# josiahbjorgaard/mca-paper

Measured on AMD Instinct MI355X. Metric: training samples/sec (fwd+bwd+opt), CMU 4-modality MCA, higher is better.
Workload: dtype bf16; 1 GPU; synthetic CMU 4-modality (MCA fcl), N=2538 D=512 L=5 H=8 F=88, lengths=full, p_drop=0.0; per_gpu_batch=32, global_batch=32, parallelism=dp1, inputs=device-resident, same batch every step, finite_checks=on (device flag, polled), attention_operands=bf16, attention_backward=bf16 one-pass, launch=hipGraph replay (one launch per step), collectives=none

## Files before the change

include/mca_hip.h:

```cpp
#ifndef MCA_HIP_H
#define MCA_HIP_H
#include <stdint.h>

#ifdef __cplusplus
extern "C" {
#endif

typedef void* mca_stream_t;

#define MCA_OK 0
#define MCA_E_BADARG (-1)
#define MCA_E_ALIGN (-2)
#define MCA_E_UNSUPPORTED (-3)
#define MCA_E_LAUNCH (-4)

const char* mca_version(void);

int mca_gemm_nt(const uint16_t* A, int64_t lda, const uint16_t* B, int64_t ldb,
                void* C, int64_t ldc, int out_bf16,
                const float* bias, const float* residual, int64_t ldres, int64_t res_period,
                int64_t M, int64_t N, int64_t K, mca_stream_t stream);

int mca_gemm_nt_cb(const uint16_t* A, int64_t lda, const uint16_t* B, int64_t ldb, uint16_t* C, int64_t cbs,
                   int64_t M, int64_t N, int64_t K, mca_stream_t stream);
// ... 5 lines not shown
int mca_gemm_nt_geglu_bwd(const uint16_t* A, int64_t lda, const uint16_t* B, int64_t ldb, const uint16_t* h,
                          uint16_t* dh, int64_t ldh, int64_t ip, int64_t M, int64_t K, mca_stream_t stream);

int mca_gemm_nt_geglu_fwd(const uint16_t* A, int64_t lda, const uint16_t* W1, int64_t ldb, uint16_t* h, int64_t ldh,
                          uint16_t* g, int64_t ldg, int64_t ip, int64_t M, int64_t K, mca_stream_t stream);

int mca_gemm_nt_geglu_fwd_saved(const uint16_t* A, int64_t lda, const uint16_t* W1, int64_t ldb, uint16_t* s, int64_t lds,
                                uint16_t* g, int64_t ldg, int64_t ip, int64_t M, int64_t K, mca_stream_t stream);
int mca_gemm_nt_geglu_bwd_saved(const uint16_t* A, int64_t lda, const uint16_t* B, int64_t ldb, const uint16_t* s,
                                uint16_t* dh, int64_t ldh, int64_t ip, int64_t M, int64_t K, mca_stream_t stream);

int mca_gemm_nt_res_lnbwd(const uint16_t* A, int64_t lda, const uint16_t* B, int64_t ldb, const float* residual, int64_t ldres,
                          const float* x, int64_t ldx, const float* mean, const float* rstd, const float* gamma,
                          float* dx, int64_t lddx, uint16_t* dx_bf16, int64_t ld_bf16, float* dgamma,
                          int64_t M, int64_t N, int64_t K, mca_stream_t stream);

int mca_gemm_tn_acc(const uint16_t* A, int64_t lda, const uint16_t* B, int64_t ldb,
                    float* C, int64_t ldc, int64_t R, int64_t N, int64_t K, mca_stream_t stream);

#define MCA_TN_MAX_GROUP 8
typedef struct mca_tn_desc {
  const uint16_t* A; int64_t lda;
  const uint16_t* B; int64_t ldb;
  float* C; int64_t ldc;
  int64_t N, K;
} mca_tn_desc;
int mca_gemm_tn_acc_group(const mca_tn_desc* d, int n, int64_t R, mca_stream_t stream);

int mca_layernorm_fwd(const float* x, int64_t ldx, const float* gamma, const float* beta,
                      const uint8_t* rowmask, const float* add, int64_t period,
// ... 310 lines not shown
```

mca-paper_amd/csrc/gemm.hip:

```cpp
#include "common.h"
#include "gemm_plan.h"
#include "gemm_tile.h"
#include "ln_rows.h"

static int num_cus() {
  static int n = 0;
  if (!n) {
    int dev = 0;
    if (hipGetDevice(&dev) != hipSuccess || hipDeviceGetAttribute(&n, hipDeviceAttributeMultiprocessorCount, dev) != hipSuccess || n <= 0) n = 256;
  }
  return n;
}

#define PS_PANELS 4
__device__ __forceinline__ void ps_tile_decode(int tile, int tiles_m, int tiles_n, int flat, int& tm, int& tn) {
  if (flat == 1) { tm = tile / tiles_n; tn = tile % tiles_n; return; }
  const int P = flat > 1 ? flat : PS_PANELS;
  const int per_group = P * tiles_n;
  const int g = tile / per_group;
  const int gh = (g + 1) * P <= tiles_m ? P : tiles_m - g * P;
  const int rem = tile - g * per_group;
  tn = rem / gh; tm = g * P + rem % gh;
}

// ... 846 lines not shown
          st4b(dx_bf16 + r1 * ld_bf16 + c, o);
        }
      }
    }
  }
  __syncthreads();
#pragma unroll
  for (int i = 0; i < 2; i++) *reinterpret_cast<float4*>(cs + wave * ROWS_N + (lane + 64 * i) * 4) = dg[i];
  __syncthreads();
  float t = cs[tid];
#pragma unroll
  for (int w = 1; w < 8; w++) t += cs[w * ROWS_N + tid];
  if (t != 0.f) atomicAdd(dgamma + tid, t);
}


template <bool DET>
__global__ __launch_bounds__(256) void gemm_tn_kernel(const u16* __restrict__ A, int64_t lda,
                                                       const u16* __restrict__ B, int64_t ldb, float* __restrict__ C,
                                                       int64_t ldc, int R, int N, int K, int tiles_k, int rows_per_split, int dbg) {
  __shared__ __attribute__((aligned(16))) u16 lds[2 * 2 * BR * 128];
  u16* As = lds;
  u16* Bs = lds + 2 * BR * 128;
  const int tn = blockIdx.x / tiles_k, tk = blockIdx.x % tiles_k;
  const int n0 = tn * 128, k0 = tk * 128;
  const int r_begin = blockIdx.y * rows_per_split;
  int r_end = r_begin + rows_per_split; if (r_end > R) r_end = R;
  if (r_begin >= r_end) return;
  const int tid = threadIdx.x, lane = tid & 63, wave = tid >> 6;
  const int wn = wave >> 1, wk = wave & 1;
// ... 401 lines not shown
}

extern "C" int mca_gemm_nt_lnres(const uint16_t* A, int64_t lda, const uint16_t* B, int64_t ldb, float* C, int64_t ldc,
                                 const float* x, int64_t ldx, const float* mean, const float* rstd, const float* gamma,
                                 int64_t M, int64_t N, int64_t K, mca_stream_t stream) {
  if (!A || !B || !C || !x || !mean || !rstd || !gamma || M <= 0 || N <= 0 || K <= 0) return MCA_E_BADARG;
  if (K % 64 || lda % 8 || ldb % 8 || ldc % 4 || ldx % 4 || (uintptr_t)A % 16 || (uintptr_t)B % 16 || (uintptr_t)C % 16 ||
      (uintptr_t)x % 16 || (uintptr_t)gamma % 16)
    return MCA_E_ALIGN;
  if (lda < K || ldb < K || ldc < N || ldx < N) return MCA_E_BADARG;
  if (!mca_nt_lnres_supported(M, N, K)) return MCA_E_UNSUPPORTED;
  const gemm_operands o = {A, lda, B, ldb, C, ldc, nullptr, x, ldx, 0, mean, rstd, gamma, (int)M, (int)K, nullptr};
  return launch(mca_plan_gemm_nt_lnres(M, N), o, stream);
}

extern "C" int mca_gemm_nt_res_lnbwd(const uint16_t* A, int64_t lda, const uint16_t* B, int64_t ldb, const float* residual, int64_t ldres,
                                     const float* x, int64_t ldx, const float* mean, const float* rstd, const float* gamma,
                                     float* dx, int64_t lddx, uint16_t* dx_bf16, int64_t ld_bf16, float* dgamma,
                                     int64_t M, int64_t N, int64_t K, mca_stream_t stream) {
  if (!A || !B || !x || !mean || !rstd || !gamma || !dx || !dx_bf16 || !dgamma || M <= 0 || N <= 0 || K <= 0) return MCA_E_BADARG;
  const int refusal = mca_nt_rows_refusal(M, N, K);
  if (refusal) return refusal;
  if (lda % 8 || ldb % 8 || ldx % 4 || lddx % 4 || ld_bf16 % 8 || (residual && ldres % 4) || (uintptr_t)A % 16 || (uintptr_t)B % 16 ||
      (uintptr_t)x % 16 || (uintptr_t)gamma % 16 || (uintptr_t)dx % 16 || (uintptr_t)dx_bf16 % 16 || (uintptr_t)residual % 16)
    return MCA_E_ALIGN;
  if (lda < K || ldb < K || ldx < N || lddx < N || ld_bf16 < N || (residual && ldres < N)) return MCA_E_BADARG;
  const mca_gemm_plan p = mca_plan_gemm_nt_res_lnbwd(M);
  return launch_kernel<gemm_nt_rows_kernel>(p, stream, A, lda, B, ldb, residual, ldres, x, ldx, mean, rstd, gamma, dx, lddx, dx_bf16, ld_bf16,
                                               dgamma, (int)M, (int)K, p.nwg);
}

static int geglu_bwd_entry(bool saved, const uint16_t* A, int64_t lda, const uint16_t* B, int64_t ldb, const uint16_t* h,
                           uint16_t* dh, int64_t ldh, int64_t ip, int64_t M, int64_t K, mca_stream_t stream) {
  if (!A || !B || !h || !dh || M <= 0 || ip <= 0 || K <= 0) return MCA_E_BADARG;
  if (K % 64 || lda % 8 || ldb % 8 || ldh % 8 || ip % 8 || (uintptr_t)A % 16 || (uintptr_t)B % 16 || (uintptr_t)h % 16 || (uintptr_t)dh % 16)
    return MCA_E_ALIGN;
  if (lda < K || ldb < K || ldh < 2 * ip) return MCA_E_BADARG;
  if (M > (1LL << 30)) return MCA_E_UNSUPPORTED;
  const gemm_operands o = {A, lda, B, ldb, dh, ldh, nullptr, reinterpret_cast<const float*>(h), ldh, 0, nullptr, nullptr, nullptr, (int)M, (int)K, nullptr};
  return launch(saved ? mca_plan_gemm_nt_geglu_bwd_saved(M, ip, K, mca_knobs, num_cus()) : mca_plan_gemm_nt_geglu_bwd(M, ip, K, mca_knobs, num_cus()),
                o, stream);
}
extern "C" int mca_gemm_nt_geglu_bwd(const uint16_t* A, int64_t lda, const uint16_t* B, int64_t ldb, const uint16_t* h,
                                     uint16_t* dh, int64_t ldh, int64_t ip, int64_t M, int64_t K, mca_stream_t stream) {
// ... 160 lines not shown
  if (!pr || !out) return MCA_E_BADARG;
  if (cus <= 0) cus = num_cus();
  switch (entry) {
    case 0: *out = mca_plan_gemm_nt(*pr, mca_knobs, cus); return MCA_OK;
    case 1:
      if (!mca_nt_lnres_supported(pr->M, pr->N, pr->K)) return MCA_E_UNSUPPORTED;
      *out = mca_plan_gemm_nt_lnres(pr->M, pr->N); return MCA_OK;
    case 2: *out = mca_plan_gemm_nt_geglu_fwd(pr->M, pr->N, pr->K, mca_knobs, cus); return MCA_OK;
    case 3: *out = mca_plan_gemm_nt_geglu_bwd(pr->M, pr->N, pr->K, mca_knobs, cus); return MCA_OK;
    case 4: *out = mca_plan_gemm_nt_geglu_fwd_saved(pr->M, pr->N, pr->K, mca_knobs, cus); return MCA_OK;
    case 5: *out = mca_plan_gemm_nt_geglu_bwd_saved(pr->M, pr->N, pr->K, mca_knobs, cus); return MCA_OK;
    case 6:
      if (pr->M <= 0 || pr->N <= 0 || pr->K <= 0) return MCA_E_BADARG;
      if (mca_nt_rows_refusal(pr->M, pr->N, pr->K)) return mca_nt_rows_refusal(pr->M, pr->N, pr->K);
      *out = mca_plan_gemm_nt_res_lnbwd(pr->M); return MCA_OK;
  }
  return MCA_E_BADARG;
}
extern "C" int mca_dbg_plan_gemm_nt_cb(int64_t M, int64_t N, int64_t K, uint64_t C, int64_t cbs, int cus, mca_gemm_plan* out) {
  if (!out || M <= 0 || N <= 0 || K <= 0) return MCA_E_BADARG;
  if (cus <= 0) cus = num_cus();
  return mca_plan_gemm_nt_cb(M, N, K, C, cbs, mca_knobs, cus, out) ? MCA_OK : MCA_E_UNSUPPORTED;
}
extern "C" const char* mca_dbg_gemm_kernel_name(int kernel) { return mca_gemm_kernel_name(kernel); }
extern "C" int mca_dbg_plan_gemm_tn(int64_t R, int64_t N, int64_t K, mca_gemm_plan* out) {
  if (!out || R <= 0 || N <= 0 || K <= 0) return MCA_E_BADARG;
  *out = mca_plan_gemm_tn(R, N, K, mca_knobs);
  return MCA_OK;
}
extern "C" int mca_dbg_plan_gemm_tn_group(const int64_t* N, const int64_t* K, int n, int64_t R, int cus, mca_tn_group_plan* out) {
// ... 22 lines not shown
```

mca-paper_amd/csrc/gemm_plan.h:

```cpp
#pragma once
#include <stdint.h>

#define BM 128
#define BN 128
#define BM2 256
#define BR 64
#define BR2 32
#define P2_STAGE (512 * 32)
#define TN2_STAGE (BR2 * 512)
#define TN2_NSTAGE 5
#define NT256_LDS_BYTES (3 * (BM2 + BN) * 64 * 2)
#define NT256LN_LDS_BYTES (NT256_LDS_BYTES + 2048)
#define NTPS_LDS_BYTES (3 * (BM2 + BN) * 64 * 2 + 16384)
#define P2_LDS_BYTES (5 * P2_STAGE * 2)
#define TN256_LDS_BYTES (3 * BR * (256 + 128) * 2)
#define TN2_LDS_BYTES (TN2_NSTAGE * TN2_STAGE * 2)

enum mca_gemm_kernel {
  MCA_GK_NONE = 0,
  MCA_GK_NT_GLDS = 1,
  MCA_GK_NT_GLDS_GEGLU_BWD = 7,
  MCA_GK_NT_256 = 8,
  MCA_GK_NT_256_PF = 14,
  MCA_GK_NT_256_LNRES = 15,
// ... 3 lines not shown
  MCA_GK_NT_PERSIST_GEGLU_FWD = 24,
  MCA_GK_NT_PERSIST256 = 25,
  MCA_GK_NT_PERSIST256_GEGLU_FWD = 26,
  MCA_GK_TN = 27,
  MCA_GK_TN_256 = 28,
  MCA_GK_TN_256X256 = 29,
  MCA_GK_TN_256X256_GROUP = 30,
  MCA_GK_COUNT = 31,
  MCA_GK_SAVED = 64,
  MCA_GK_NT_GLDS_GEGLU_BWD_SAVED = MCA_GK_SAVED + MCA_GK_NT_GLDS_GEGLU_BWD,
  MCA_GK_NT_256_GEGLU_BWD_SAVED = MCA_GK_SAVED + MCA_GK_NT_256_GEGLU_BWD,
  MCA_GK_NT_PERSIST_GEGLU_BWD_SAVED = MCA_GK_SAVED + MCA_GK_NT_PERSIST_GEGLU_BWD,
  MCA_GK_NT_PERSIST_GEGLU_FWD_SAVED = MCA_GK_SAVED + MCA_GK_NT_PERSIST_GEGLU_FWD,
  MCA_GK_NT_PERSIST256_GEGLU_FWD_SAVED = MCA_GK_SAVED + MCA_GK_NT_PERSIST256_GEGLU_FWD,
  MCA_GK_NT_ROWS_LNBWD = 128,
  MCA_GK_NT_PERSIST256_CB = 256
};

static inline const char* mca_gemm_kernel_name(int k) {
  static const char* const names[MCA_GK_COUNT] = {
      "none",
      "gemm_nt_glds_kernel<false,0,64,0>", "gemm_nt_glds_kernel<false,1,64,0>", "gemm_nt_glds_kernel<false,2,64,0>",
      "gemm_nt_glds_kernel<true,0,64,0>", "gemm_nt_glds_kernel<true,1,64,0>", "gemm_nt_glds_kernel<true,2,64,0>",
      "gemm_nt_glds_kernel<true,0,64,1>",
      "gemm_nt_256_kernel<false,0,0,0>", "gemm_nt_256_kernel<false,1,0,0>", "gemm_nt_256_kernel<false,2,0,0>",
      "gemm_nt_256_kernel<true,0,0,0>", "gemm_nt_256_kernel<true,1,0,0>", "gemm_nt_256_kernel<true,2,0,0>",
      "gemm_nt_256_kernel<false,1,1,0>", "gemm_nt_256_kernel<false,1,1,2>", "gemm_nt_256_kernel<true,0,0,1>",
      "gemm_nt_persist_kernel<0,false>", "gemm_nt_persist_kernel<0,true>", "gemm_nt_persist_kernel<1,false>",
      "gemm_nt_persist_kernel<1,true>", "gemm_nt_persist_kernel<2,false>", "gemm_nt_persist_kernel<2,true>",
      "gemm_nt_persist_kernel<3,false>", "gemm_nt_persist_kernel<4,false>",
      "gemm_nt_persist256_kernel<false>", "gemm_nt_persist256_kernel<true>",
      "gemm_tn_kernel", "gemm_tn_256_kernel", "gemm_tn_256x256_kernel", "gemm_tn_256x256_group_kernel"};
  switch (k) {
    case MCA_GK_NT_GLDS_GEGLU_BWD_SAVED: return "gemm_nt_glds_kernel<true,0,64,3>";
    case MCA_GK_NT_256_GEGLU_BWD_SAVED: return "gemm_nt_256_kernel<true,0,0,3>";
    case MCA_GK_NT_PERSIST_GEGLU_BWD_SAVED: return "gemm_nt_persist_kernel<5,false>";
    case MCA_GK_NT_PERSIST_GEGLU_FWD_SAVED: return "gemm_nt_persist_kernel<6,false>";
    case MCA_GK_NT_PERSIST256_GEGLU_FWD_SAVED: return "gemm_nt_persist256_kernel<true,true>";
    case MCA_GK_NT_ROWS_LNBWD: return "gemm_nt_rows_kernel";
    case MCA_GK_NT_PERSIST256_CB: return "gemm_nt_persist256_kernel<false,false,true>";
  }
  return k >= 0 && k < MCA_GK_COUNT ? names[k] : "?";
}

struct mca_gemm_plan {
  int kernel;
  int grid_x, grid_y, block, lds_bytes;
  int n;
  int tiles_n, nwg;
  int tiles_k, rows_per_split;
  int dbg;
};

#define MCA_NT_BIG_M 2048
// ... 124 lines not shown
#define ROWS_CS_LD (ROWS_N + 4)
#define ROWS_LDS_BYTES (ROWS_NSTAGE * ROWS_STAGE * 2)
#define MCA_NT_ROWS_MIN_K (ROWS_NSTAGE * ROWS_BK)

static inline int mca_nt_rows_refusal(int64_t M, int64_t N, int64_t K) {
  if (N != ROWS_N || M > (1LL << 30)) return -3;
  if (K % ROWS_BK) return -2;
  if (K < MCA_NT_ROWS_MIN_K) return -3;
  return 0;
}
static inline mca_gemm_plan mca_plan_gemm_nt_res_lnbwd(int64_t M) {
  mca_gemm_plan pl = {};
  pl.kernel = MCA_GK_NT_ROWS_LNBWD;
  pl.n = ROWS_N; pl.tiles_n = 1; pl.nwg = (int)((M + ROWS_BM - 1) / ROWS_BM);
  pl.grid_x = pl.nwg; pl.grid_y = 1; pl.block = 512; pl.lds_bytes = ROWS_LDS_BYTES;
  return pl;
}

#define MCA_TN_BIG_N 512
#define MCA_TN_BIG_R 4096
#define MCA_TN_HUGE_MIN_K 512
#define MCA_TN_HUGE_MIN_TILES 8

static inline mca_gemm_plan mca_plan_gemm_tn(int64_t R, int64_t N, int64_t K, const int* knobs) {
  const bool big = N >= MCA_TN_BIG_N && R >= MCA_TN_BIG_R && knobs[5] != 1;
  const bool huge = big && K >= MCA_TN_HUGE_MIN_K && knobs[5] != 2 && ((N + 255) / 256) * ((K + 255) / 256) >= MCA_TN_HUGE_MIN_TILES;
  const int tiles_k = (int)(huge ? (K + 255) / 256 : (K + 127) / 128);
  const int tiles_n = big ? (int)((N + 255) / 256) : (int)((N + 127) / 128);
  const int tiles = tiles_n * tiles_k;
  int64_t splits = big ? (tiles <= 16 ? 256 / tiles : 512 / tiles) : (tiles <= 32 ? 512 / tiles : 1024 / tiles);
// ... 191 lines not shown
```

mca-paper_amd/engine.py:

```python
from __future__ import annotations

import os

import ctypes as C
import weakref
import math
from typing import Callable, Dict, List, Optional

import numpy as np
import torch

from . import attention, hip
from .attention import AttnGrads, AttnKeys, AttnOperands, _OnePassSched, _Sched, _dev
from .encoder_steps import FLAG_INDEX_RANGE, step_for
from .hip import AttnFp8BwdOperands, AttnFp8Operands, LossTerm, call, ptr, stream_ptr

LN_EPS = 1e-5
FWD_BQ, FWD_BK = 128, 64
BWD_BQ = 64


FLAG_CACHE_MISMATCH = 8


def _pad_to(x: int, m: int) -> int:
    return (x + m - 1) // m * m


def debug_options() -> dict:
    opts = {"overlap_wgrad": None, "group_wgrad": True, "mask_mfma": True, "dkv_keys": 128, "lazy_softmax": True,
            "onepass": None, "deterministic": False, "geglu_saved": True, "ln_rows": True,
            "qkv_hm": True}
    for item in filter(None, os.environ.get("MCA_DEBUG", "").split(",")):
        k, _, v = item.partition("=")
        k = k.strip()
        if k not in opts:
            raise ValueError(f"MCA_DEBUG: unknown switch '{k}' (known: {sorted(opts)})")
        opts[k] = int(v) if k == "dkv_keys" else (v.strip() not in ("0", "", "false"))
    return opts


def _ln_bwd_args(dy, ldy, x, gamma, mean, rstd, rows, cols, dgamma, dbeta=None, rowmask=None, dx=None, dx_bf16=None,
                 y_bstride=0, period=0, dxsum=None):
    return (ptr(dy), ldy, y_bstride, period, ptr(x), x.stride(0), ptr(gamma), ptr(mean), ptr(rstd),
            ptr(rowmask), ptr(dx), dx.stride(0) if dx is not None else 0, ptr(dx_bf16),
            dx_bf16.stride(0) if dx_bf16 is not None else 0, ptr(dgamma), ptr(dbeta), ptr(dxsum), rows, cols)
# ... 31 lines not shown
        self.enc_steps = [step_for(self, name, mi, model.encoders[name]) for mi, name in enumerate(model.modality_types)]
        self._alloc_weights()
        self._ws: Dict[int, dict] = {}
        self._weights_version = -1
        self.grad_bucket_hook: Optional[Callable[[int, int], None]] = None
        self.gather_hook: Optional[Callable] = None
        self.check_finite = True
        self.finite_flag = torch.zeros(1, dtype=torch.int32, device=self.device)
        self._flag_host = torch.zeros(1, dtype=torch.int32).pin_memory()
        self._flag_event: Optional[torch.cuda.Event] = None
        self.fuse_geglu_bwd = True
        self.geglu_saved_factors = bool(self.dbg["geglu_saved"])
        self._mod_shifts = torch.arange(len(model.modality_types), dtype=torch.int32, device=self.device)
        self.fuse_ln_residual = True
        self.fuse_ln_rows = bool(self.dbg["ln_rows"])
        self.rows_only = False
        self.overlap_wgrad = self.dbg["overlap_wgrad"]
        self.group_wgrad = self.dbg["group_wgrad"]
        self._deterministic = bool(self.dbg["deterministic"])
        self._captured = weakref.WeakSet()
        self._mdrop: Optional[dict] = None
        self._mdrop_counter: Optional[torch.Tensor] = None
        self.dropout_rank = 0

    def _flatten_parameters(self):
        m = self.model
        order: List[torch.nn.Parameter] = []
        marks: List[int] = []
        order += [m.loss.loss_fn.logit_scale]
        pool_kv_late = not self.eao and self.L > 0
# ... 229 lines not shown
        arr = (hip.CastDesc * len(self._cast_list))(*self._cast_list)
        self._cast_n = len(self._cast_list)
        self._cast_table = torch.frombuffer(bytearray(bytes(arr)), dtype=torch.uint8).to(self.device)
        call("mca_cast_pad_bf16_multi", ptr(self._cast_table), self._cast_n, stream_ptr())
        self._weights_version = v

    def workspace(self, b: int) -> dict:
        if b in self._ws:
            return self._ws[b]
        D, N, H, Ip, R, dev = self.D, self.N, self.H, self.Ip, self.R, self.device
        T = b * N
        f32 = lambda *s: torch.empty(*s, dtype=torch.float32, device=dev)
        bf = lambda *s: torch.empty(*s, dtype=torch.bfloat16, device=dev)
        u8 = lambda *s: torch.empty(*s, dtype=torch.uint8, device=dev)
        ws = dict(b=b, T=T, gen=0)
        ws["x"] = [f32(T, D) for _ in range(self.L + 1)]
        ws["layers"] = [dict(x1=f32(T, D), m1=f32(T), r1=f32(T), m2=f32(T), r2=f32(T), xn_b=bf(T, D), qkv=bf(T, 3 * D),
                             o=bf(T, D), lse=f32(b, H, N), x1n_b=bf(T, D), h=bf(T, 2 * Ip), g=bf(T, Ip),
                             dxo_b=bf(T, D), dx1_b=bf(T, D), dh=bf(T, 2 * Ip), dqkv=bf(T, 3 * D),
                             h_holds=None,
                             qkv_hm=False)
                        for _ in range(self.L)]
        ws["xn"], ws["x1n"] = f32(T, D), f32(T, D)
        ws["mf"], ws["rf"] = f32(T), f32(T)
        ws["t_b"], ws["kvp"] = (None, None) if self.eao else (bf(T, D), bf(T, 2 * D))
        ws["rt_b"], ws["qp"], ws["op"], ws["lse_p"] = bf(R, D), bf(R, D), bf(b * R, D), f32(b, H, R)
        ws["pooled"] = f32(b * R, D)
        if self.eao:
            ws["seg_counts"] = torch.zeros(b, R, dtype=torch.int32, device=dev)
        ws["vmean"], ws["dvmean"], ws["delta"], ws["delta_p"] = torch.zeros(b, D, dtype=torch.float32, device=dev), f32(b, D), f32(b, H, N), f32(b, H, R)
# ... 252 lines not shown
        if self.eao:
            pad2 = ws["padding"].view(b, N)
            for src, dst, n in self.st.copies:
                call("mca_rows_copy_add", x0.data_ptr() + src * D * 4, N * D, x0.data_ptr() + dst * D * 4, N * D, n, D, b, 0, stream_ptr())
                pad2[:, dst:dst + n].copy_(pad2[:, src:src + n])
        ws["present_cur"] = present
        bits = ((present[:, None] >> self._mod_shifts) & 1).to(torch.bool)
        return {name: bits[:, mi] for mi, name in enumerate(m.modality_types)}

    def ln_in_gemm(self, T: int) -> bool:
        return self.fuse_ln_residual and T >= 2048 and self.D % 128 == 0 and self.D >= 512 and self.Ip >= 512

    def ln_rows_backward(self, T: int) -> bool:
        return self.fuse_ln_rows and self.ln_in_gemm(T) and self.D == 512 and not self._deterministic and not self.eao

    def _gemm_ln_bwd(self, A, B, K, residual, x, gamma, mean, rstd, dgamma, dx, dx_bf16, T):
        D = self.D
        if hip.PROFILE is not None:
            hip.set_tag(f"{T}x{D}x{K} f32{' +res' if residual is not None else ''}")
        call("mca_gemm_nt_res_lnbwd", ptr(A), A.stride(0), ptr(B), B.stride(0), ptr(residual), residual.stride(0) if residual is not None else 0,
             ptr(x), x.stride(0), ptr(mean), ptr(rstd), ptr(gamma), ptr(dx), dx.stride(0), ptr(dx_bf16), dx_bf16.stride(0), ptr(dgamma),
             T, D, K, stream_ptr(), flops=2.0 * T * D * K, profile_as="mca_gemm_nt")
        if hip.PROFILE is not None:
            hip.set_tag("")

    def forward_trunk(self, ws):
        m, D, N, H, Ip, R, b, T = self.model, self.D, self.N, self.H, self.Ip, self.R, ws["b"], ws["T"]
        call("mca_build_keyinfo", ptr(ws["padding"]), ptr(self.kgroup), ptr(ws["keyinfo"]), ptr(ws["kflags"]), b, N,
             self.nk_pad, stream_ptr())
        if ws["khot"] is not None:
            call("mca_build_keyhot", ptr(ws["keyinfo"]), ptr(ws["khot"]), b, self.nk_pad, stream_ptr())
        ln_in_gemm = self.ln_in_gemm(T)
        saved = self.geglu_saved_factors and self.fuse_geglu_bwd
        ff1 = "mca_gemm_nt_geglu_fwd_saved" if saved else "mca_gemm_nt_geglu_fwd"
        qkv_hm = self.qkv_head_major(ws)
# ... 159 lines not shown
        self.attn_backward(*self.pool_attention(ws), ws)
        ws["dqp_sum"].zero_()
        self._reduce_rows(ws, ptr(ws["dqp32"]), D, R * D, R, ptr(ws["dqp_sum"]), D, b * R, D)
        call("mca_f32_to_bf16", ptr(ws["dqp_sum"]), D, ptr(ws["dqp_b"]), D, R, D, 1.0, stream_ptr())
        self.gemm_nt(ws["dqp_b"], self.wp["qT"], ws["drt"], R, D, D)
        self._reduce_rows(ws, ptr(ws["drt"]), D, R * D, R, ptr(G(m.return_tokens)), D, R, D)
        on_side(lambda: tn(ws["dqp_b"], ws["rt_b"], G(ap.to_q.weight), R, D, D))
        pool_kv = (ws["dkvp"], ws["t_b"], G(ap.to_kv.weight), 2 * D, D)
        if not (self.L > 0 and self.group_wgrad and T >= 4096):
            on_side(lambda pk=pool_kv: tn(pk[0], pk[1], pk[2], T, 2 * D, D))
            pool_kv = None
        dx, dx_other = ws["dxa"], ws["dxb"]
        top = ws["layers"][self.L - 1]["dxo_b"] if self.L else ws["dx_b"]
        if self.ln_rows_backward(T):
            self._gemm_ln_bwd(ws["dkvp"], self.wp["kvT"], 2 * D, None, ws["x"][self.L], m.norm.gamma, ws["mf"], ws["rf"], G(m.norm.gamma),
                              dx_other, top, T)
        else:
            self.gemm_nt(ws["dkvp"], self.wp["kvT"], dx, T, D, 2 * D)
            self._ln_bwd(ws, dx, D, ws["x"][self.L], m.norm.gamma, ws["mf"], ws["rf"], T, D, G(m.norm.gamma), dx=dx_other, dx_bf16=top)
        dx, dx_other = dx_other, dx
        on_side(lambda: bucket_ready(0))
        self._backward_layers_and_encoders(ws, dx, dx_other, bucket_ready, on_side, extra_top=pool_kv)

    def _backward_part_eao(self, ws, dpool, bucket_ready, on_side):
        m, D, N, R, b, T = self.model, self.D, self.N, self.R, ws["b"], ws["T"]
        dx, dx_other = ws["dxa"], ws["dxb"]
        call("mca_segment_mean_bwd", ptr(dpool), ptr(ws["padding"]), ptr(self.kgroup), ptr(ws["seg_counts"]), R, ptr(dx), b, N, D,
             stream_ptr())
        top = ws["layers"][self.L - 1]["dxo_b"] if self.L else ws["dx_b"]
        self._ln_bwd(ws, dx, D, ws["x"][self.L], m.norm.gamma, ws["mf"], ws["rf"], T, D, self.grad_of(m.norm.gamma), dx=dx_other, dx_bf16=top)
        dx, dx_other = dx_other, dx
# ... 14 lines not shown
                on_side(lambda dxo=dxo, a=a, ly=ly: tn(dxo, a["g"], G(ly.ff.feedforward[2].weight), T, D, I))
            saved = self.geglu_saved_factors and self.fuse_geglu_bwd
            assert a["h_holds"] == ("s" if saved else "h"), \
                f"layer {i}: the forward left {a['h_holds']!r} in the GEGLU buffer; geglu_saved_factors / fuse_geglu_bwd changed since"
            if self.fuse_geglu_bwd:
                call("mca_gemm_nt_geglu_bwd_saved" if saved else "mca_gemm_nt_geglu_bwd", ptr(dxo), D, ptr(w["w2T"]), D,
                     ptr(a["h"]), ptr(dh), 2 * Ip, Ip, T, D, stream_ptr(), flops=2.0 * T * Ip * D, profile_as="mca_gemm_nt_geglu_bwd")
            else:
                self.gemm_nt(dxo, w["w2T"], ws["dg"], T, Ip, D)
                call("mca_geglu_bwd", ptr(ws["dg"]), ptr(a["h"]), ptr(dh), T, Ip, stream_ptr())
            gw1 = G(ly.ff.feedforward[0].weight)
            if not grouped:
                on_side(lambda dh=dh, a=a, gw1=gw1: (tn(dh, a["x1n_b"], gw1, T, I, D), tn(dh[:, Ip:], a["x1n_b"], gw1[I:], T, I, D)))
            rows = self.ln_rows_backward(T)
            if rows:
                self._gemm_ln_bwd(dh, w["w1T"], 2 * Ip, dx, a["x1"], g, a["m2"], a["r2"], G(g), dx, dx1, T)
            else:
                self.gemm_nt(dh, w["w1T"], dx_other, T, D, 2 * Ip, residual=dx)
                self._ln_bwd(ws, dx_other, D, a["x1"], g, a["m2"], a["r2"], T, D, G(g), dx=dx, dx_bf16=dx1)
            if not grouped:
                on_side(lambda dx1=dx1, a=a, ly=ly: tn(dx1, a["o"], G(ly.attn.to_out.weight), T, D, D))
            ws["do_hm"] = a["qkv_hm"] and self.backward_plan(ws, b, self.N).form == "onepass"
            (self.gemm_nt_cb if ws["do_hm"] else self.gemm_nt)(dx1, w["oT"], ws["do"], T, D, D)
            self.attn_backward(*self.layer_attention(ws, i), ws)
            gq = G(ly.attn.to_q.weight)
            assert G(ly.attn.to_kv.weight).data_ptr() == gq.data_ptr() + D * D * 4
            if grouped:
                gw2, gwo = G(ly.ff.feedforward[2].weight), G(ly.attn.to_out.weight)
                extra = [extra_top] if (bi == 0 and extra_top is not None) else []
                on_side(lambda dqkv=dqkv, dh=dh, dxo=dxo, dx1=dx1, a=a, gq=gq, gw1=gw1, gw2=gw2, gwo=gwo, extra=extra: self._tn_group(
                    ws, [(dqkv, a["xn_b"], gq, 3 * D, D), (dh, a["x1n_b"], gw1, I, D), (dh[:, Ip:], a["x1n_b"], gw1[I:], I, D),
                     (dxo, a["g"], gw2, D, I), (dx1, a["o"], gwo, D, D)] + extra, T))
            else:
                on_side(lambda dqkv=dqkv, a=a, gq=gq: tn(dqkv, a["xn_b"], gq, T, 3 * D, D))
            if rows:
                self._gemm_ln_bwd(dqkv, w["qkvT"], 3 * D, dx, ws["x"][i], g, a["m1"], a["r1"], G(g), dx, below, T)
            else:
                self.gemm_nt(dqkv, w["qkvT"], dx_other, T, D, 3 * D, residual=dx)
                self._ln_bwd(ws, dx_other, D, ws["x"][i], g, a["m1"], a["r1"], T, D, G(g), dx=dx, dx_bf16=below)
            on_side(lambda bi=bi: bucket_ready(bi + 1))
        if self.eao:
            for src, dst, n in self.st.copies:
                call("mca_rows_copy_add", dx.data_ptr() + dst * D * 4, N * D, dx.data_ptr() + src * D * 4, N * D, n, D, b, 1, stream_ptr())
        if self.F:
            self._reduce_rows(ws, dx.data_ptr() + (N - self.F) * D * 4, D, N * D, self.F, ptr(G(m.fusion_tokens)), D, b * self.F, D)
        for step in self.enc_steps:
            step.backward(ws, dx, on_side)
        on_side(lambda: bucket_ready(len(self.bucket_bounds) - 1))

    def model_forward(self, batch, no_loss=False):
        with hip.cached_stream():
# ... 156 lines not shown
```

mca-paper_amd/hip.py:

```python
from __future__ import annotations

import ctypes as C
import os
from typing import Optional

import torch

_HERE = os.path.dirname(os.path.abspath(__file__))
LIB_PATH = os.environ.get("MCA_HIP_LIB") or os.path.join(_HERE, "libmca_hip.so")

_ERR = {-1: "bad argument", -2: "misaligned pointer / leading dimension", -3: "unsupported size", -4: "launch failed"}


class MCAHipError(RuntimeError):
    pass


class LossTerm(C.Structure):
    _fields_ = [("slot_a", C.c_int32), ("slot_b", C.c_int32), ("and_bits", C.c_uint32), ("or_bits", C.c_uint32)]


class CastDesc(C.Structure):
    _fields_ = [("src", C.c_void_p), ("dst", C.c_void_p), ("lds", C.c_int64), ("rows", C.c_int64), ("cols", C.c_int64),
                ("ldd", C.c_int64), ("rows_pad", C.c_int64), ("cols_pad", C.c_int64), ("transpose", C.c_int32), ("scale", C.c_float)]
# ... 151 lines not shown
    _fields_ = [("grouped", C.c_int), ("launch", GemmPlan), ("part", TnPartition)]


class TnDetPlan(C.Structure):
    _fields_ = [("launch", GemmPlan), ("slots", C.c_int), ("slot_stride", C.c_int64), ("scratch_floats", C.c_int64)]


class TnGroupDetPlan(C.Structure):
    _fields_ = [("plan", TnGroupPlan), ("slots", C.c_int), ("slot_stride", C.c_int64), ("scratch_floats", C.c_int64)]


PLAN_NT, PLAN_LNRES, PLAN_GEGLU_FWD, PLAN_GEGLU_BWD, PLAN_GEGLU_FWD_SAVED, PLAN_GEGLU_BWD_SAVED = range(6)
GK_SAVED = 64
PLAN_RES_LNBWD = 6
GK_NT_ROWS_LNBWD = 128
GK_NT_PERSIST256_CB = 256


class LnFwdProblem(C.Structure):
    _fields_ = [("rows", C.c_int64), ("cols", C.c_int32), ("cols_pad", C.c_int32)] + \
               [(f, C.c_int64) for f in ("ldx", "ldy", "y_bstride", "ld_bf16", "period")] + \
               [(f, C.c_uint64) for f in ("x", "gamma", "beta", "rowmask", "add", "y", "y_bf16")]


class LnFwdPlan(C.Structure):
    _fields_ = [("form", C.c_int32), ("width", C.c_int32), ("grid_x", C.c_int64), ("passes", C.c_int64)]


class LnBwdProblem(C.Structure):
    _fields_ = [("rows", C.c_int64), ("cols", C.c_int32), ("pad_", C.c_int32)] + \
# ... 13 lines not shown
SIGNATURES = {
    "mca_version": (C.c_char_p, []),
    "mca_flag_to_host": (_I, [_P, _P, _P]),
    "mca_build_keyhot": (_I, [_P, _P, _I, _I, _P]),
    "mca_rows_copy_add": (_I, [_P, _I64, _P, _I64, _I64, _I, _I, _I, _P]),
    "mca_segment_mean_fwd": (_I, [_P, _P, _P, _I, _P, _P, _I, _I, _I, _P]),
    "mca_segment_mean_bwd": (_I, [_P, _P, _P, _P, _I, _P, _I, _I, _I, _P]),
    "mca_gemm_nt": (_I, [_P, _I64, _P, _I64, _P, _I64, _I, _P, _P, _I64, _I64, _I64, _I64, _I64, _P]),
    "mca_gemm_nt_cb": (_I, [_P, _I64, _P, _I64, _P, _I64, _I64, _I64, _I64, _P]),
    "mca_gemm_nt_geglu_bwd": (_I, [_P, _I64, _P, _I64, _P, _P, _I64, _I64, _I64, _I64, _P]),
    "mca_gemm_nt_lnres": (_I, [_P, _I64, _P, _I64, _P, _I64, _P, _I64, _P, _P, _P, _I64, _I64, _I64, _P]),
    "mca_gemm_nt_geglu_fwd": (_I, [_P, _I64, _P, _I64, _P, _I64, _P, _I64, _I64, _I64, _I64, _P]),
    "mca_gemm_nt_geglu_fwd_saved": (_I, [_P, _I64, _P, _I64, _P, _I64, _P, _I64, _I64, _I64, _I64, _P]),
    "mca_gemm_nt_geglu_bwd_saved": (_I, [_P, _I64, _P, _I64, _P, _P, _I64, _I64, _I64, _I64, _P]),
    "mca_gemm_nt_res_lnbwd": (_I, [_P, _I64, _P, _I64, _P, _I64, _P, _I64, _P, _P, _P, _P, _I64, _P, _I64, _P, _I64, _I64, _I64, _P]),
    "mca_geglu_fwd_saved": (_I, [_P, _P, _I64, _I, _P]),
    "mca_geglu_bwd_saved": (_I, [_P, _P, _P, _I64, _I, _P]),
    "mca_gemm_tn_acc": (_I, [_P, _I64, _P, _I64, _P, _I64, _I64, _I64, _I64, _P]),
    "mca_gemm_tn_acc_group": (_I, [_P, _I, _I64, _P]),
    "mca_layernorm_fwd": (_I, [_P, _I64, _P, _P, _P, _P, _I64, _P, _I64, _I64, _P, _I64, _I, _P, _P, _I64, _I, _F, _P]),
    "mca_layernorm_bwd": (_I, [_P, _I64, _I64, _I64, _P, _I64, _P, _P, _P, _P, _P, _I64, _P, _I64, _P, _P, _P, _I64, _I, _P]),
    "mca_geglu_fwd": (_I, [_P, _P, _I64, _I, _P]),
    "mca_geglu_bwd": (_I, [_P, _P, _P, _I64, _I, _P]),
    "mca_cast_pad_bf16": (_I, [_P, _I64, _I64, _I64, _P, _I64, _I64, _I64, _I, _P]),
    "mca_cast_pad_bf16_multi": (_I, [_P, _I, _P]),
    "mca_f32_to_bf16": (_I, [_P, _I64, _P, _I64, _I64, _I64, _F, _P]),
    "mca_bcast_rows": (_I, [_P, _I64, _P, _I64, _I64, _I64, _I64, _I, _P]),
    "mca_reduce_rows": (_I, [_P, _I64, _I64, _I64, _P, _I64, _I64, _I, _P]),
    "mca_embedding_renorm": (_I, [_P, _I64, _I, _F, _P]),
    "mca_embedding_lookup": (_I, [_P, _I64, _I, _F, _P, _I, _I64, _I64, _P, _P, _I64, _I64, _I, _P, _P, _I, _P]),
# ... 223 lines not shown
```

Before: 1761 samples/s.

## Add 160-row tile variant of fused GEMM+LayerNorm-backward kernel chosen by wave-quantization cost

Adds a gemm_nt_rows160_kernel that processes 160 rows per workgroup (five 32-row MFMA sub-tiles, with waves 0-1 loading the extra A rows) for the fused GEMM + residual + LayerNorm backward. A planner compares per-CU row cost for 128- versus 160-row tiles given M and the CU count, and picks the taller tile when it reduces wave-quantization tail. The engine caches this choice per K and routes to the new entry point. The trade-off is more accumulator registers and LDS per block, which may lower occupancy.

```diff
diff --git a/include/mca_hip.h b/include/mca_hip.h
--- a/include/mca_hip.h
+++ b/include/mca_hip.h
@@ -43,6 +43,10 @@
                           const float* x, int64_t ldx, const float* mean, const float* rstd, const float* gamma,
                           float* dx, int64_t lddx, uint16_t* dx_bf16, int64_t ld_bf16, float* dgamma,
                           int64_t M, int64_t N, int64_t K, mca_stream_t stream);
+int mca_gemm_nt_res_lnbwd_tall(const uint16_t* A, int64_t lda, const uint16_t* B, int64_t ldb, const float* residual, int64_t ldres,
+                               const float* x, int64_t ldx, const float* mean, const float* rstd, const float* gamma,
+                               float* dx, int64_t lddx, uint16_t* dx_bf16, int64_t ld_bf16, float* dgamma,
+                               int64_t M, int64_t N, int64_t K, mca_stream_t stream);
 
 int mca_gemm_tn_acc(const uint16_t* A, int64_t lda, const uint16_t* B, int64_t ldb,
                     float* C, int64_t ldc, int64_t R, int64_t N, int64_t K, mca_stream_t stream);
diff --git a/mca-paper_amd/csrc/gemm.hip b/mca-paper_amd/csrc/gemm.hip
--- a/mca-paper_amd/csrc/gemm.hip
+++ b/mca-paper_amd/csrc/gemm.hip
@@ -884,6 +884,183 @@
   if (t != 0.f) atomicAdd(dgamma + tid, t);
 }
 
+__global__ __launch_bounds__(512) void gemm_nt_rows160_kernel(
+    const u16* __restrict__ A, int64_t lda, const u16* __restrict__ B, int64_t ldb, const float* residual, int64_t ldres,
+    const float* __restrict__ x, int64_t ldx, const float* __restrict__ mean_in, const float* __restrict__ rstd_in,
+    const float* __restrict__ gamma, float* dx, int64_t lddx, u16* __restrict__ dx_bf16, int64_t ld_bf16, float* __restrict__ dgamma,
+    int M, int K, int nwg) {
+  extern __shared__ __attribute__((aligned(16))) u16 lds2[];
+  constexpr unsigned STAGE_BYTES = ROWS160_STAGE * 2;
+  const int tid = threadIdx.x, lane = tid & 63, wave = tid >> 6;
+  const int l31 = lane & 31, lh = lane >> 5;
+  const bool six = __builtin_amdgcn_readfirstlane(wave) < 2;
+  const int nkt = K / ROWS_BK;
+  const int m0 = xcd_remap(blockIdx.x, nwg) * ROWS160_BM;
+  const unsigned lds_base = lds_addr(lds2);
+
+  unsigned fa_addr[5], fb_addr[2];
+#pragma unroll
+  for (int i = 0; i < 5; i++) { const int r = i * 32 + l31; fa_addr[i] = lds_base + (unsigned)(r * 64 + ((lh ^ gl_sw<32>(r)) << 4)); }
+#pragma unroll
+  for (int j = 0; j < 2; j++) { const int r = wave * 64 + j * 32 + l31; fb_addr[j] = lds_base + (unsigned)(ROWS160_BM * 64) + (unsigned)(r * 64 + ((lh ^ gl_sw<32>(r)) << 4)); }
+
+  const u16* ga[2];
+  const u16* gb[4];
+#pragma unroll
+  for (int i = 0; i < 2; i++) {
+    const int p = (i * 8 + (i ? wave & 1 : wave)) * 64 + lane, r = p >> 2, c = (p & 3) ^ gl_sw<32>(r);
+    int ra = m0 + r; if (ra > M - 1) ra = M - 1;
+    ga[i] = A + (int64_t)ra * lda + c * 8;
+  }
+#pragma unroll
+  for (int i = 0; i < 4; i++) {
+    const int p = (i * 8 + wave) * 64 + lane, r = p >> 2, c = (p & 3) ^ gl_sw<32>(r);
+    gb[i] = B + (int64_t)r * ldb + c * 8;
+  }
+  auto stage = [&](int k0, int st) {
+    u16* base = lds2 + st * ROWS160_STAGE;
+    lds_dma16(ga[0] + k0, base + wave * 512);
+    if (six) lds_dma16(ga[1] + k0, base + (8 + wave) * 512);
+#pragma unroll
+    for (int i = 0; i < 4; i++) lds_dma16(gb[i] + k0, base + ROWS160_BM * ROWS_BK + (i * 8 + wave) * 512);
+  };
+
+  f32x16 acc[5][2];
+#pragma unroll
+  for (int i = 0; i < 5; i++)
+#pragma unroll
+    for (int j = 0; j < 2; j++)
+#pragma unroll
+      for (int r = 0; r < 16; r++) acc[i][j][r] = 0.f;
+  stage(0, 0); stage(ROWS_BK, 1); stage(2 * ROWS_BK, 2);
+  u32x4v fa[2][5], fb[2][2];
+#define R160_RA(KS, I, SO) NT_DSREAD(fa[KS][I], (fa_addr[I] + (SO)) ^ (32u * (KS))); T256_SB
+#define R160_RB(KS, J, SO) NT_DSREAD(fb[KS][J], (fb_addr[J] + (SO)) ^ (32u * (KS))); T256_SB
+#define R160_MM(KS, I, J) acc[I][J] = __builtin_amdgcn_mfma_f32_32x32x16_bf16(*reinterpret_cast<const bf16x8*>(&fa[KS][I]), \
+                                                                              *reinterpret_cast<const bf16x8*>(&fb[KS][J]), acc[I][J], 0, 0, 0); T256_SB
+#define R160_FIRST_READS R160_RA(0, 0, 0u) R160_RB(0, 0, 0u) R160_RB(0, 1, 0u) R160_RA(0, 1, 0u) R160_RA(0, 2, 0u) R160_RA(0, 3, 0u) R160_RA(0, 4, 0u)
+#define R160_GROUP_READING(KS, KN, SO, MID)                                                                                       \
+  R160_MM(KS, 0, 0) MID R160_RA(KN, 0, SO) R160_MM(KS, 0, 1) R160_RA(KN, 1, SO) R160_MM(KS, 1, 0) R160_RA(KN, 2, SO)                \
+  R160_MM(KS, 1, 1) R160_RA(KN, 3, SO) R160_MM(KS, 2, 0) R160_RB(KN, 0, SO) R160_MM(KS, 2, 1) R160_RB(KN, 1, SO)                    \
+  R160_MM(KS, 3, 0) R160_RA(KN, 4, SO) R160_MM(KS, 3, 1) R160_MM(KS, 4, 0) R160_MM(KS, 4, 1)
+#define R160_GROUP(KS) R160_MM(KS, 0, 0) R160_MM(KS, 0, 1) R160_MM(KS, 1, 0) R160_MM(KS, 1, 1) R160_MM(KS, 2, 0) R160_MM(KS, 2, 1) \
+  R160_MM(KS, 3, 0) R160_MM(KS, 3, 1) R160_MM(KS, 4, 0) R160_MM(KS, 4, 1)
+  if (six) ps_wait_vm<12>(); else ps_wait_vm<10>();
+  __builtin_amdgcn_s_barrier();
+  T256_SB
+  R160_FIRST_READS
+  int slot = 0;
+  for (int kt = 0; kt + 1 < nkt; kt++) {
+    const unsigned so = (unsigned)slot * STAGE_BYTES;
+    const int nxt = slot == 2 ? 0 : slot + 1;
+    asm volatile("s_waitcnt lgkmcnt(0)" ::: "memory"); T256_SB
+    R160_GROUP_READING(0, 1, so, )
+    if (kt + 2 < nkt) {
+      if (six) asm volatile("s_waitcnt vmcnt(6) lgkmcnt(0)" ::: "memory");
+      else asm volatile("s_waitcnt vmcnt(5) lgkmcnt(0)" ::: "memory");
+    } else asm volatile("s_waitcnt vmcnt(0) lgkmcnt(0)" ::: "memory");
+    __builtin_amdgcn_s_barrier();
+    T256_SB
+    const unsigned son = (unsigned)nxt * STAGE_BYTES;
+    const bool fetch = kt + 3 < nkt;
+    R160_GROUP_READING(1, 0, son, if (fetch) stage((kt + 3) * ROWS_BK, slot); T256_SB)
+    slot = nxt;
+  }
+  {
+    const unsigned so = (unsigned)slot * STAGE_BYTES;
+    asm volatile("s_waitcnt lgkmcnt(0)" ::: "memory"); T256_SB
+    R160_GROUP_READING(0, 1, so, )
+    asm volatile("s_waitcnt lgkmcnt(0)" ::: "memory"); T256_SB
+    R160_GROUP(1)
+  }
+#undef R160_RA
+#undef R160_RB
+#undef R160_MM
+#undef R160_FIRST_READS
+#undef R160_GROUP_READING
+#undef R160_GROUP
+  __syncthreads();
+
+  float* cs = reinterpret_cast<float*>(lds2);
+  float4 gm[2], dg[2];
+#pragma unroll
+  for (int i = 0; i < 2; i++) { gm[i] = *reinterpret_cast<const float4*>(gamma + (lane + 64 * i) * 4); dg[i] = make_float4(0.f, 0.f, 0.f, 0.f); }
+  const float inv_cols = 1.f / (float)ROWS_N;
+  auto ld4 = [](const float* p) { const f32x4 t = __builtin_nontemporal_load(reinterpret_cast<const f32x4*>(p)); return make_float4(t[0], t[1], t[2], t[3]); };
+  auto st4 = [](float* p, const float4& o) { __builtin_nontemporal_store(f32x4{o.x, o.y, o.z, o.w}, reinterpret_cast<f32x4*>(p)); };
+  auto st4b = [](u16* p, const float4& o) { const uint2 pk = ln_pack4bf(o); __builtin_nontemporal_store(u32x2v{pk.x, pk.y}, reinterpret_cast<u32x2v*>(p)); };
+#pragma unroll
+  for (int p = 0; p < 5; p++) {
+    float4 xq[2][2][2], rq[2][2][2];
+#pragma unroll
+    for (int q = 0; q < 2; q++) {
+      const int mrow = m0 + p * 32 + wave * 4 + q * 2;
+      const int64_t r0 = mrow < M ? mrow : M - 1, r1 = mrow + 1 < M ? mrow + 1 : r0;
+#pragma unroll
+      for (int i = 0; i < 2; i++) {
+        const int c = (lane + 64 * i) * 4;
+        xq[q][0][i] = ld4(x + r0 * ldx + c); xq[q][1][i] = ld4(x + r1 * ldx + c);
+        if (residual) { rq[q][0][i] = ld4(residual + r0 * ldres + c); rq[q][1][i] = ld4(residual + r1 * ldres + c); }
+        else { rq[q][0][i] = make_float4(0.f, 0.f, 0.f, 0.f); rq[q][1][i] = make_float4(0.f, 0.f, 0.f, 0.f); }
+      }
+    }
+    if (p) __syncthreads();
+#pragma unroll
+    for (int j = 0; j < 2; j++)
+#pragma unroll
+      for (int rr = 0; rr < 16; rr++) cs[acc_row(rr, lh) * ROWS_CS_LD + wave * 64 + j * 32 + l31] = acc[p][j][rr];
+    __syncthreads();
+#pragma unroll
+    for (int q = 0; q < 2; q++) {
+      const int lr = wave * 4 + q * 2;
+      const int mrow = m0 + p * 32 + lr;
+      if (mrow >= M) continue;
+      const bool two = mrow + 1 < M;
+      const int64_t r0 = mrow, r1 = two ? r0 + 1 : r0;
+      const float* ca = cs + lr * ROWS_CS_LD;
+      const float* cb = cs + (two ? lr + 1 : lr) * ROWS_CS_LD;
+      float4 xa[2], xb[2], da[2], db[2];
+#pragma unroll
+      for (int i = 0; i < 2; i++) {
+        const int c = (lane + 64 * i) * 4;
+        xa[i] = xq[q][0][i]; da[i] = *reinterpret_cast<const float4*>(ca + c);
+        xb[i] = xq[q][1][i]; db[i] = *reinterpret_cast<const float4*>(cb + c);
+      }
+      if (residual) {
+#pragma unroll
+        for (int i = 0; i < 2; i++) {
+          const float4 ta = rq[q][0][i], tb = rq[q][1][i];
+          da[i].x += ta.x; da[i].y += ta.y; da[i].z += ta.z; da[i].w += ta.w;
+          db[i].x += tb.x; db[i].y += tb.y; db[i].z += tb.z; db[i].w += tb.w;
+        }
+      }
+      const float ma = mean_in[r0], ra = rstd_in[r0], mb = mean_in[r1], rb = rstd_in[r1];
+      float s1a, s2a, s1b, s2b;
+      ln_bwd_rows_stats<2>(xa, xb, da, db, gm, dg, ma, ra, mb, rb, two, inv_cols, s1a, s2a, s1b, s2b);
+#pragma unroll
+      for (int i = 0; i < 2; i++) {
+        const int c = (lane + 64 * i) * 4;
+        float4 o = ln_bwd_row_dx(da[i], xa[i], ra, s1a, s2a);
+        st4(dx + r0 * lddx + c, o);
+        st4b(dx_bf16 + r0 * ld_bf16 + c, o);
+        if (two) {
+          o = ln_bwd_row_dx(db[i], xb[i], rb, s1b, s2b);
+          st4(dx + r1 * lddx + c, o);
+          st4b(dx_bf16 + r1 * ld_bf16 + c, o);
+        }
+      }
+    }
+  }
+  __syncthreads();
+#pragma unroll
+  for (int i = 0; i < 2; i++) *reinterpret_cast<float4*>(cs + wave * ROWS_N + (lane + 64 * i) * 4) = dg[i];
+  __syncthreads();
+  float t = cs[tid];
+#pragma unroll
+  for (int w = 1; w < 8; w++) t += cs[w * ROWS_N + tid];
+  if (t != 0.f) atomicAdd(dgamma + tid, t);
+}
+
 
 template <bool DET>
 __global__ __launch_bounds__(256) void gemm_tn_kernel(const u16* __restrict__ A, int64_t lda,
@@ -1315,10 +1492,9 @@
   return launch(mca_plan_gemm_nt_lnres(M, N), o, stream);
 }
 
-extern "C" int mca_gemm_nt_res_lnbwd(const uint16_t* A, int64_t lda, const uint16_t* B, int64_t ldb, const float* residual, int64_t ldres,
-                                     const float* x, int64_t ldx, const float* mean, const float* rstd, const float* gamma,
-                                     float* dx, int64_t lddx, uint16_t* dx_bf16, int64_t ld_bf16, float* dgamma,
-                                     int64_t M, int64_t N, int64_t K, mca_stream_t stream) {
+static int res_lnbwd_refusal(const uint16_t* A, int64_t lda, const uint16_t* B, int64_t ldb, const float* residual, int64_t ldres,
+                             const float* x, int64_t ldx, const float* mean, const float* rstd, const float* gamma,
+                             float* dx, int64_t lddx, uint16_t* dx_bf16, int64_t ld_bf16, float* dgamma, int64_t M, int64_t N, int64_t K) {
   if (!A || !B || !x || !mean || !rstd || !gamma || !dx || !dx_bf16 || !dgamma || M <= 0 || N <= 0 || K <= 0) return MCA_E_BADARG;
   const int refusal = mca_nt_rows_refusal(M, N, K);
   if (refusal) return refusal;
@@ -1326,9 +1502,34 @@
       (uintptr_t)x % 16 || (uintptr_t)gamma % 16 || (uintptr_t)dx % 16 || (uintptr_t)dx_bf16 % 16 || (uintptr_t)residual % 16)
     return MCA_E_ALIGN;
   if (lda < K || ldb < K || ldx < N || lddx < N || ld_bf16 < N || (residual && ldres < N)) return MCA_E_BADARG;
+  return MCA_OK;
+}
+extern "C" int mca_gemm_nt_res_lnbwd(const uint16_t* A, int64_t lda, const uint16_t* B, int64_t ldb, const float* residual, int64_t ldres,
+                                     const float* x, int64_t ldx, const float* mean, const float* rstd, const float* gamma,
+                                     float* dx, int64_t lddx, uint16_t* dx_bf16, int64_t ld_bf16, float* dgamma,
+                                     int64_t M, int64_t N, int64_t K, mca_stream_t stream) {
+  const int rc = res_lnbwd_refusal(A, lda, B, ldb, residual, ldres, x, ldx, mean, rstd, gamma, dx, lddx, dx_bf16, ld_bf16, dgamma, M, N, K);
+  if (rc != MCA_OK) return rc;
   const mca_gemm_plan p = mca_plan_gemm_nt_res_lnbwd(M);
   return launch_kernel<gemm_nt_rows_kernel>(p, stream, A, lda, B, ldb, residual, ldres, x, ldx, mean, rstd, gamma, dx, lddx, dx_bf16, ld_bf16,
                                                dgamma, (int)M, (int)K, p.nwg);
+}
+extern "C" int mca_gemm_nt_res_lnbwd_tall(const uint16_t* A, int64_t lda, const uint16_t* B, int64_t ldb, const float* residual, int64_t ldres,
+                                          const float* x, int64_t ldx, const float* mean, const float* rstd, const float* gamma,
+                                          float* dx, int64_t lddx, uint16_t* dx_bf16, int64_t ld_bf16, float* dgamma,
+                                          int64_t M, int64_t N, int64_t K, mca_stream_t stream) {
+  const int rc = res_lnbwd_refusal(A, lda, B, ldb, residual, ldres, x, ldx, mean, rstd, gamma, dx, lddx, dx_bf16, ld_bf16, dgamma, M, N, K);
+  if (rc != MCA_OK) return rc;
+  const mca_gemm_plan p = mca_plan_gemm_nt_res_lnbwd_tall(M, mca_knobs, num_cus());
+  switch (p.kernel) {
+    case MCA_GK_NT_ROWS_LNBWD:
+      return launch_kernel<gemm_nt_rows_kernel>(p, stream, A, lda, B, ldb, residual, ldres, x, ldx, mean, rstd, gamma, dx, lddx, dx_bf16, ld_bf16,
+                                                   dgamma, (int)M, (int)K, p.nwg);
+    case MCA_GK_NT_ROWS160_LNBWD:
+      return launch_kernel<gemm_nt_rows160_kernel>(p, stream, A, lda, B, ldb, residual, ldres, x, ldx, mean, rstd, gamma, dx, lddx, dx_bf16,
+                                                      ld_bf16, dgamma, (int)M, (int)K, p.nwg);
+  }
+  return MCA_E_LAUNCH;
 }
 
 static int geglu_bwd_entry(bool saved, const uint16_t* A, int64_t lda, const uint16_t* B, int64_t ldb, const uint16_t* h,
@@ -1519,6 +1720,10 @@
       if (pr->M <= 0 || pr->N <= 0 || pr->K <= 0) return MCA_E_BADARG;
       if (mca_nt_rows_refusal(pr->M, pr->N, pr->K)) return mca_nt_rows_refusal(pr->M, pr->N, pr->K);
       *out = mca_plan_gemm_nt_res_lnbwd(pr->M); return MCA_OK;
+    case 7:
+      if (pr->M <= 0 || pr->N <= 0 || pr->K <= 0) return MCA_E_BADARG;
+      if (mca_nt_rows_refusal(pr->M, pr->N, pr->K)) return mca_nt_rows_refusal(pr->M, pr->N, pr->K);
+      *out = mca_plan_gemm_nt_res_lnbwd_tall(pr->M, mca_knobs, cus); return MCA_OK;
   }
   return MCA_E_BADARG;
 }
diff --git a/mca-paper_amd/csrc/gemm_plan.h b/mca-paper_amd/csrc/gemm_plan.h
--- a/mca-paper_amd/csrc/gemm_plan.h
+++ b/mca-paper_amd/csrc/gemm_plan.h
@@ -41,6 +41,7 @@
   MCA_GK_NT_PERSIST_GEGLU_FWD_SAVED = MCA_GK_SAVED + MCA_GK_NT_PERSIST_GEGLU_FWD,
   MCA_GK_NT_PERSIST256_GEGLU_FWD_SAVED = MCA_GK_SAVED + MCA_GK_NT_PERSIST256_GEGLU_FWD,
   MCA_GK_NT_ROWS_LNBWD = 128,
+  MCA_GK_NT_ROWS160_LNBWD = 160,
   MCA_GK_NT_PERSIST256_CB = 256
 };
 
@@ -65,6 +66,7 @@
     case MCA_GK_NT_PERSIST_GEGLU_FWD_SAVED: return "gemm_nt_persist_kernel<6,false>";
     case MCA_GK_NT_PERSIST256_GEGLU_FWD_SAVED: return "gemm_nt_persist256_kernel<true,true>";
     case MCA_GK_NT_ROWS_LNBWD: return "gemm_nt_rows_kernel";
+    case MCA_GK_NT_ROWS160_LNBWD: return "gemm_nt_rows160_kernel";
     case MCA_GK_NT_PERSIST256_CB: return "gemm_nt_persist256_kernel<false,false,true>";
   }
   return k >= 0 && k < MCA_GK_COUNT ? names[k] : "?";
@@ -219,6 +221,30 @@
   pl.kernel = MCA_GK_NT_ROWS_LNBWD;
   pl.n = ROWS_N; pl.tiles_n = 1; pl.nwg = (int)((M + ROWS_BM - 1) / ROWS_BM);
   pl.grid_x = pl.nwg; pl.grid_y = 1; pl.block = 512; pl.lds_bytes = ROWS_LDS_BYTES;
+  return pl;
+}
+
+#define ROWS160_BM 160
+#define ROWS160_STAGE ((ROWS160_BM + ROWS_N) * ROWS_BK)
+#define ROWS160_LDS_BYTES (ROWS_NSTAGE * ROWS160_STAGE * 2)
+#define MCA_KNOB_ROWS_HEIGHT 15
+
+static inline int64_t mca_nt_rows_cost(int64_t M, int h, int cus) {
+  const int64_t tiles = (M + h - 1) / h;
+  return (tiles + cus - 1) / cus * h;
+}
+static inline int mca_nt_rows_height(int64_t M, int cus) {
+  if (cus < 1) cus = 1;
+  return mca_nt_rows_cost(M, ROWS160_BM, cus) < mca_nt_rows_cost(M, ROWS_BM, cus) ? ROWS160_BM : ROWS_BM;
+}
+static inline mca_gemm_plan mca_plan_gemm_nt_res_lnbwd_tall(int64_t M, const int* knobs, int cus) {
+  const int forced = knobs[MCA_KNOB_ROWS_HEIGHT];
+  const int h = forced == 1 ? ROWS_BM : forced == 2 ? ROWS160_BM : mca_nt_rows_height(M, cus);
+  if (h == ROWS_BM) return mca_plan_gemm_nt_res_lnbwd(M);
+  mca_gemm_plan pl = {};
+  pl.kernel = MCA_GK_NT_ROWS160_LNBWD;
+  pl.n = ROWS_N; pl.tiles_n = 1; pl.nwg = (int)((M + ROWS160_BM - 1) / ROWS160_BM);
+  pl.grid_x = pl.nwg; pl.grid_y = 1; pl.block = 512; pl.lds_bytes = ROWS160_LDS_BYTES;
   return pl;
 }
 
diff --git a/mca-paper_amd/engine.py b/mca-paper_amd/engine.py
--- a/mca-paper_amd/engine.py
+++ b/mca-paper_amd/engine.py
@@ -29,7 +29,7 @@
 
 def debug_options() -> dict:
     opts = {"overlap_wgrad": None, "group_wgrad": True, "mask_mfma": True, "dkv_keys": 128, "lazy_softmax": True,
-            "onepass": None, "deterministic": False, "geglu_saved": True, "ln_rows": True,
+            "onepass": None, "deterministic": False, "geglu_saved": True, "ln_rows": True, "ln_rows_tall": True,
             "qkv_hm": True}
     for item in filter(None, os.environ.get("MCA_DEBUG", "").split(",")):
         k, _, v = item.partition("=")
@@ -91,6 +91,7 @@
         self._mod_shifts = torch.arange(len(model.modality_types), dtype=torch.int32, device=self.device)
         self.fuse_ln_residual = True
         self.fuse_ln_rows = bool(self.dbg["ln_rows"])
+        self.ln_rows_tall = bool(self.dbg["ln_rows_tall"])
         self.rows_only = False
         self.overlap_wgrad = self.dbg["overlap_wgrad"]
         self.group_wgrad = self.dbg["group_wgrad"]
@@ -350,6 +351,7 @@
         bf = lambda *s: torch.empty(*s, dtype=torch.bfloat16, device=dev)
         u8 = lambda *s: torch.empty(*s, dtype=torch.uint8, device=dev)
         ws = dict(b=b, T=T, gen=0)
+        ws["ln_rows_tall"] = {}
         ws["x"] = [f32(T, D) for _ in range(self.L + 1)]
         ws["layers"] = [dict(x1=f32(T, D), m1=f32(T), r1=f32(T), m2=f32(T), r2=f32(T), xn_b=bf(T, D), qkv=bf(T, 3 * D),
                              o=bf(T, D), lse=f32(b, H, N), x1n_b=bf(T, D), h=bf(T, 2 * Ip), g=bf(T, Ip),
@@ -632,11 +634,23 @@
     def ln_rows_backward(self, T: int) -> bool:
         return self.fuse_ln_rows and self.ln_in_gemm(T) and self.D == 512 and not self._deterministic and not self.eao
 
-    def _gemm_ln_bwd(self, A, B, K, residual, x, gamma, mean, rstd, dgamma, dx, dx_bf16, T):
-        D = self.D
+    def ln_rows_tall_form(self, ws, K: int) -> bool:
+        if not self.ln_rows_tall:
+            return False
+        tall = ws["ln_rows_tall"]
+        if K not in tall:
+            pl = hip.GemmPlan()
+            cus = torch.cuda.get_device_properties(self.device).multi_processor_count
+            rc = hip.lib().mca_dbg_plan_gemm_nt(hip.PLAN_RES_LNBWD_TALL, C.byref(hip.NtProblem(M=ws["T"], N=self.D, K=K)), cus, C.byref(pl))
+            tall[K] = rc == 0 and pl.kernel == hip.GK_NT_ROWS160_LNBWD
+        return tall[K]
+
+    def _gemm_ln_bwd(self, A, B, K, residual, x, gamma, mean, rstd, dgamma, dx, dx_bf16, ws):
+        D, T = self.D, ws["T"]
         if hip.PROFILE is not None:
             hip.set_tag(f"{T}x{D}x{K} f32{' +res' if residual is not None else ''}")
-        call("mca_gemm_nt_res_lnbwd", ptr(A), A.stride(0), ptr(B), B.stride(0), ptr(residual), residual.stride(0) if residual is not None else 0,
+        call("mca_gemm_nt_res_lnbwd_tall" if self.ln_rows_tall_form(ws, K) else "mca_gemm_nt_res_lnbwd",
+             ptr(A), A.stride(0), ptr(B), B.stride(0), ptr(residual), residual.stride(0) if residual is not None else 0,
              ptr(x), x.stride(0), ptr(mean), ptr(rstd), ptr(gamma), ptr(dx), dx.stride(0), ptr(dx_bf16), dx_bf16.stride(0), ptr(dgamma),
              T, D, K, stream_ptr(), flops=2.0 * T * D * K, profile_as="mca_gemm_nt")
         if hip.PROFILE is not None:
@@ -826,7 +840,7 @@
         top = ws["layers"][self.L - 1]["dxo_b"] if self.L else ws["dx_b"]
         if self.ln_rows_backward(T):
             self._gemm_ln_bwd(ws["dkvp"], self.wp["kvT"], 2 * D, None, ws["x"][self.L], m.norm.gamma, ws["mf"], ws["rf"], G(m.norm.gamma),
-                              dx_other, top, T)
+                              dx_other, top, ws)
         else:
             self.gemm_nt(ws["dkvp"], self.wp["kvT"], dx, T, D, 2 * D)
             self._ln_bwd(ws, dx, D, ws["x"][self.L], m.norm.gamma, ws["mf"], ws["rf"], T, D, G(m.norm.gamma), dx=dx_other, dx_bf16=top)
@@ -871,7 +885,7 @@
                 on_side(lambda dh=dh, a=a, gw1=gw1: (tn(dh, a["x1n_b"], gw1, T, I, D), tn(dh[:, Ip:], a["x1n_b"], gw1[I:], T, I, D)))
             rows = self.ln_rows_backward(T)
             if rows:
-                self._gemm_ln_bwd(dh, w["w1T"], 2 * Ip, dx, a["x1"], g, a["m2"], a["r2"], G(g), dx, dx1, T)
+                self._gemm_ln_bwd(dh, w["w1T"], 2 * Ip, dx, a["x1"], g, a["m2"], a["r2"], G(g), dx, dx1, ws)
             else:
                 self.gemm_nt(dh, w["w1T"], dx_other, T, D, 2 * Ip, residual=dx)
                 self._ln_bwd(ws, dx_other, D, a["x1"], g, a["m2"], a["r2"], T, D, G(g), dx=dx, dx_bf16=dx1)
@@ -891,7 +905,7 @@
             else:
                 on_side(lambda dqkv=dqkv, a=a, gq=gq: tn(dqkv, a["xn_b"], gq, T, 3 * D, D))
             if rows:
-                self._gemm_ln_bwd(dqkv, w["qkvT"], 3 * D, dx, ws["x"][i], g, a["m1"], a["r1"], G(g), dx, below, T)
+                self._gemm_ln_bwd(dqkv, w["qkvT"], 3 * D, dx, ws["x"][i], g, a["m1"], a["r1"], G(g), dx, below, ws)
             else:
                 self.gemm_nt(dqkv, w["qkvT"], dx_other, T, D, 3 * D, residual=dx)
                 self._ln_bwd(ws, dx_other, D, ws["x"][i], g, a["m1"], a["r1"], T, D, G(g), dx=dx, dx_bf16=below)
diff --git a/mca-paper_amd/hip.py b/mca-paper_amd/hip.py
--- a/mca-paper_amd/hip.py
+++ b/mca-paper_amd/hip.py
@@ -189,6 +189,9 @@
 GK_SAVED = 64
 PLAN_RES_LNBWD = 6
 GK_NT_ROWS_LNBWD = 128
+PLAN_RES_LNBWD_TALL = 7
+GK_NT_ROWS160_LNBWD = 160
+KNOB_ROWS_HEIGHT = 15
 GK_NT_PERSIST256_CB = 256
 
 
@@ -232,6 +235,7 @@
     "mca_gemm_nt_geglu_fwd_saved": (_I, [_P, _I64, _P, _I64, _P, _I64, _P, _I64, _I64, _I64, _I64, _P]),
     "mca_gemm_nt_geglu_bwd_saved": (_I, [_P, _I64, _P, _I64, _P, _P, _I64, _I64, _I64, _I64, _P]),
     "mca_gemm_nt_res_lnbwd": (_I, [_P, _I64, _P, _I64, _P, _I64, _P, _I64, _P, _P, _P, _P, _I64, _P, _I64, _P, _I64, _I64, _I64, _P]),
+    "mca_gemm_nt_res_lnbwd_tall": (_I, [_P, _I64, _P, _I64, _P, _I64, _P, _I64, _P, _P, _P, _P, _I64, _P, _I64, _P, _I64, _I64, _I64, _P]),
     "mca_geglu_fwd_saved": (_I, [_P, _P, _I64, _I, _P]),
     "mca_geglu_bwd_saved": (_I, [_P, _P, _P, _I64, _I, _P]),
     "mca_gemm_tn_acc": (_I, [_P, _I64, _P, _I64, _P, _I64, _I64, _I64, _I64, _P]),
```

Measured after the change: 1799 samples/s (median of 6 runs). 1.02x the previous value.
